# akamiru/bce

Measured on AMD Instinct MI355X. Metric: MB/s compressed, higher is better.
Workload: dtype u8/u32 integer

## Files before the change

bce_amd/csrc/k1_bwt.hip:

```cpp
#include <stdlib.h>

#include <utility>

#include "common.h"
#include "scan_util.h"

namespace bce {

#ifndef K1_ACT_TENTHS
#define K1_ACT_TENTHS 6
#endif

constexpr int K1_T = 256;

constexpr uint32_t K1_MAXB = 1024;
struct K1Plan { uint32_t nb, per_block; };
static K1Plan k1_plan(uint32_t n) {
  const uint32_t chunk = 2048;
  uint32_t chunks = (uint32_t)(((uint64_t)n + chunk - 1) / chunk);
  if (!chunks) chunks = 1;
  uint32_t nb = chunks < K1_MAXB ? chunks : K1_MAXB;
  uint32_t cpb = (chunks + nb - 1) / nb;
  nb = (chunks + cpb - 1) / cpb;
  return {nb, cpb * chunk};
// ... 21 lines not shown
#pragma unroll
    for (uint32_t b = 0; b < 3; ++b) {
      uint64_t q = i + b;
      if (q >= m) q -= m;
      k = (k << 9) | (q == m - 1u ? 0u : (uint32_t)T[q] + 1u);
    }
    keys[i] = k;
    vals[i] = (uint32_t)i;
  }
}

__global__ __launch_bounds__(K1_T) void k1_gather_prev_kernel(const uint32_t *__restrict__ sa,
                                                              const uint32_t *__restrict__ rank, uint32_t n,
                                                              uint32_t h, uint32_t *__restrict__ keys,
                                                              uint32_t *__restrict__ vals) {
  for (uint64_t j = (uint64_t)blockIdx.x * K1_T + threadIdx.x; j < n; j += (uint64_t)gridDim.x * K1_T) {
    const uint32_t q = sa[j];
    const uint32_t p = q >= h ? q - h : q + (n - h);
    vals[j] = p;
    keys[j] = rank[p];
  }
}

__global__ __launch_bounds__(K1_T) void k1_gather_next_kernel(const uint32_t *__restrict__ sa,
                                                              const uint32_t *__restrict__ rank, uint32_t n,
                                                              uint32_t h, uint32_t *__restrict__ k2) {
  for (uint64_t j = (uint64_t)blockIdx.x * K1_T + threadIdx.x; j < n; j += (uint64_t)gridDim.x * K1_T) {
    const uint64_t q = (uint64_t)sa[j] + h;
    k2[j] = rank[q >= n ? q - n : q];
  }
}

__global__ __launch_bounds__(K1_T) void k1_heads_kernel(const uint32_t *__restrict__ k1,
                                                        const uint32_t *__restrict__ k2, uint32_t n,
                                                        uint32_t per_block, uint32_t *__restrict__ nrk,
                                                        uint32_t *__restrict__ blockmax, uint32_t *__restrict__ groups) {
  const uint64_t beg = (uint64_t)blockIdx.x * per_block;
  uint64_t end = beg + per_block;
  if (end > n) end = n;
  uint32_t mx = 0, cnt = 0;
  for (uint64_t j = beg + threadIdx.x; j < end; j += K1_T) {
    bool head = (j == 0);
    if (!head) {
      head = k1[j] != k1[j - 1];
      if (!head && k2) head = k2[j] != k2[j - 1];
    }
    nrk[j] = head ? (uint32_t)j : 0u;
    if (head) { mx = (uint32_t)j; ++cnt; }
  }
  mx = block_reduce_max<K1_T>(mx);
  cnt = block_reduce_sum<K1_T>(cnt);
  if (threadIdx.x == 0) {
    blockmax[blockIdx.x] = mx;
    if (cnt) atomicAdd(groups, cnt);
  }
}

__global__ __launch_bounds__(K1_T) void k1_apply_kernel(const uint32_t *__restrict__ nrk,
                                                        const uint32_t *__restrict__ blockmax, uint32_t n,
                                                        uint32_t per_block, const uint32_t *__restrict__ sa,
                                                        uint32_t *__restrict__ rank) {
  uint32_t c = 0;
  for (uint32_t b = threadIdx.x; b < blockIdx.x; b += K1_T) { const uint32_t v = blockmax[b]; c = c > v ? c : v; }
  uint32_t carry = block_reduce_max<K1_T>(c);
  const uint64_t beg = (uint64_t)blockIdx.x * per_block;
  uint64_t end = beg + per_block;
  if (end > n) end = n;
  for (uint64_t base = beg; base < end; base += K1_T) {
    const uint64_t j = base + threadIdx.x;
    const bool valid = j < end;
    const uint32_t v = valid ? nrk[j] : 0u;
    uint32_t tot;
    uint32_t inc = block_incl_scan_max<K1_T>(v, &tot);
    inc = inc > carry ? inc : carry;
    if (valid) rank[sa[j]] = inc;
    carry = carry > tot ? carry : tot;
  }
}

#ifndef K1_PART_MIN
#define K1_PART_MIN (1u << 27)
#endif

__global__ __launch_bounds__(K1_T) void k1_headidx_kernel(const uint32_t *__restrict__ nrk, const uint32_t *__restrict__ blockmax, uint32_t n,
                                                          uint32_t per_block, uint32_t *__restrict__ hv) {
  uint32_t c = 0;
  for (uint32_t b = threadIdx.x; b < blockIdx.x; b += K1_T) { const uint32_t v = blockmax[b]; c = c > v ? c : v; }
  uint32_t carry = block_reduce_max<K1_T>(c);
  const uint64_t beg = (uint64_t)blockIdx.x * per_block;
  uint64_t end = beg + per_block;
  if (end > n) end = n;
  for (uint64_t base = beg; base < end; base += K1_T) {
    const uint64_t j = base + threadIdx.x;
    const bool valid = j < end;
    const uint32_t v = valid ? nrk[j] : 0u;
    uint32_t tot;
    uint32_t inc = block_incl_scan_max<K1_T>(v, &tot);
    inc = inc > carry ? inc : carry;
    if (valid) hv[j] = inc;
    carry = carry > tot ? carry : tot;
  }
}
__global__ __launch_bounds__(K1_T) void k1_scatter32_kernel(const uint32_t *__restrict__ key, const uint32_t *__restrict__ val, uint32_t m,
                                                            uint32_t limit, uint32_t *__restrict__ dst) {
  for (uint64_t i = (uint64_t)blockIdx.x * K1_T + threadIdx.x; i < m; i += (uint64_t)gridDim.x * K1_T) {
    const uint32_t k = key[i];
    if (k < limit) dst[k] = val[i];
  }
}
__global__ __launch_bounds__(K1_T) void k1_seg_pairs_kernel(const uint32_t *__restrict__ vs, const uint8_t *__restrict__ flag, uint8_t defer, uint32_t m,
                                                            uint32_t *__restrict__ key) {
  for (uint64_t i = (uint64_t)blockIdx.x * K1_T + threadIdx.x; i < m; i += (uint64_t)gridDim.x * K1_T)
    key[i] = (flag[i] & defer) ? 0xFFFFFFFFu : vs[i];
}
__global__ __launch_bounds__(K1_T) void k1_bwt_kernel(const uint8_t *__restrict__ T, const uint32_t *__restrict__ sa,
                                                      uint32_t n, uint8_t *__restrict__ bwt) {
  for (uint64_t j = (uint64_t)blockIdx.x * K1_T + threadIdx.x; j < n; j += (uint64_t)gridDim.x * K1_T) {
    const uint32_t q = sa[j];
    bwt[j] = T[q ? q - 1 : n - 1];
  }
}

__global__ __launch_bounds__(K1_T) void k1_offset_kernel(const uint32_t *__restrict__ rank, uint32_t n,
                                                         uint32_t *__restrict__ out) {
  uint32_t best = 0xFFFFFFFFu;
  for (uint64_t p = (uint64_t)blockIdx.x * K1_T + threadIdx.x; p < n; p += (uint64_t)gridDim.x * K1_T)
    if (rank[p] == 0 && (uint32_t)p < best) best = (uint32_t)p;
#pragma unroll
  for (int o = 32; o > 0; o >>= 1) { const uint32_t t = __shfl_xor(best, o); best = best < t ? best : t; }
  if ((threadIdx.x & 63u) == 0 && best != 0xFFFFFFFFu) atomicMin(out, best);
}


template <int PASS>
__global__ __launch_bounds__(K1_T) void k1_active_kernel(const uint32_t *__restrict__ nrk,
                                                         const uint32_t *__restrict__ src, uint32_t m,
                                                         uint32_t per_block, uint32_t nb, uint32_t *__restrict__ blockcnt,
                                                         uint32_t *__restrict__ out, uint32_t *__restrict__ total, uint32_t mark = 0,
                                                         const uint32_t *__restrict__ sa_in = nullptr, uint32_t *__restrict__ vout = nullptr) {
  const uint64_t beg = (uint64_t)blockIdx.x * per_block;
  uint64_t end = beg + per_block;
  if (end > m) end = m;
  auto keep = [&](uint64_t i) -> bool {
    const bool h0 = i == 0 || nrk[i] != 0;
    const bool h1 = i + 1 >= m || nrk[i + 1] != 0;
    return !(h0 && h1);
  };
  if (PASS == 0) {
    uint32_t c = 0;
    for (uint64_t i = beg + threadIdx.x; i < end; i += K1_T) c += keep(i) ? 1u : 0u;
    c = block_reduce_sum<K1_T>(c);
    if (threadIdx.x == 0) blockcnt[blockIdx.x] = c;
  } else {
    uint32_t b = 0, a = 0;
    for (uint32_t k = threadIdx.x; k < nb; k += K1_T) { const uint32_t v = blockcnt[k]; a += v; if (k < blockIdx.x) b += v; }
    uint32_t base = block_reduce_sum<K1_T>(b);
    const uint32_t all = block_reduce_sum<K1_T>(a);
    if (blockIdx.x == 0 && threadIdx.x == 0) *total = all;
    for (uint64_t c0 = beg; c0 < end; c0 += K1_T) {
      const uint64_t i = c0 + threadIdx.x;
      const bool k = i < end && keep(i);
      uint32_t tot;
      const uint32_t ex = block_excl_scan_sum<K1_T>(k ? 1u : 0u, &tot);
      if (k) {
        out[base + ex] = (src ? src[i] : (uint32_t)i) | ((mark && (i == 0 || nrk[i] != 0)) ? 0x80000000u : 0u);
        if (vout) vout[base + ex] = sa_in[i];
      }
      base += tot;
    }
  }
}

__global__ __launch_bounds__(K1_T) void k1_act_gather_kernel(const uint32_t *__restrict__ A, const uint32_t *__restrict__ sa,
                                                             const uint32_t *__restrict__ rank, uint32_t n, uint32_t m,
                                                             uint32_t h, uint32_t *__restrict__ keys,
                                                             uint32_t *__restrict__ vals) {
  for (uint64_t i = (uint64_t)blockIdx.x * K1_T + threadIdx.x; i < m; i += (uint64_t)gridDim.x * K1_T) {
    const uint32_t p = sa[A[i]];
    const uint64_t q = (uint64_t)p + h;
    vals[i] = p;
    keys[i] = rank[q >= n ? q - n : q];
  }
}
__global__ __launch_bounds__(K1_T) void k1_act_group_kernel(const uint32_t *__restrict__ vals,
                                                            const uint32_t *__restrict__ rank, uint32_t m,
// ... 278 lines not shown
      }
      if (big) {
        if (w < SEG_CH) { flag[i] = KF_DEFER; ++ndef; }
      } else if (g0 >= SEG_CAP && g0 < SEG_CAP + SEG_CH) {
        mine[it] = true; gs[it] = g0 - SEG_CAP; ge[it] = g1 - SEG_CAP;
      }
    }
  }
#pragma unroll
  for (int it = 0; it < EPT; ++it) if (mine[it]) sfx[it] = V[base + it * SEG_T + (int)tid];
#pragma unroll
  for (int it = 0; it < EPT; ++it)
    if (mine[it]) {
      uint64_t q = (uint64_t)sfx[it] + h;
      if (q >= n) q -= n;
      k2[it] = rank[q];
    }
#pragma unroll
  for (int it = 0; it < EPT; ++it) if (mine[it]) K[it * SEG_T + (int)tid] = k2[it];
  if (ndef) atomicAdd(&s_defer, ndef);
  __syncthreads();
  int pos[EPT];
#pragma unroll
  for (int it = 0; it < EPT; ++it) {
    pos[it] = 0;
    if (mine[it]) {
      const int w = it * SEG_T + (int)tid;
      const uint32_t kw = k2[it];
      uint32_t r = 0;
      {
        int t = gs[it];
        const int e = w;
        for (; t < e && (t & 3); ++t) r += K[t] <= kw ? 1u : 0u;
        for (; t + 4 <= e; t += 4) {
          const uint4 v = *reinterpret_cast<const uint4 *>(&K[t]);
          r += (v.x <= kw ? 1u : 0u) + (v.y <= kw ? 1u : 0u) + (v.z <= kw ? 1u : 0u) + (v.w <= kw ? 1u : 0u);
        }
        for (; t < e; ++t) r += K[t] <= kw ? 1u : 0u;
      }
      {
        int t = w + 1;
        const int e = ge[it];
        for (; t < e && (t & 3); ++t) r += K[t] < kw ? 1u : 0u;
        for (; t + 4 <= e; t += 4) {
          const uint4 v = *reinterpret_cast<const uint4 *>(&K[t]);
          r += (v.x < kw ? 1u : 0u) + (v.y < kw ? 1u : 0u) + (v.z < kw ? 1u : 0u) + (v.w < kw ? 1u : 0u);
        }
        for (; t < e; ++t) r += K[t] < kw ? 1u : 0u;
      }
      pos[it] = gs[it] + (int)r;
    }
  }
  __syncthreads();
#pragma unroll
  for (int it = 0; it < EPT; ++it) if (mine[it]) { K[pos[it]] = k2[it]; S[pos[it]] = sfx[it]; }
  __syncthreads();
#pragma unroll
  for (int it = 0; it < EPT; ++it) {
    const int w = it * SEG_T + (int)tid;
    if ((w & ~63) < cntw) {
      const bool nh = mine[it] && (w == gs[it] || K[w] != K[w - 1]);
      const uint64_t bal = __ballot(nh);
      if (lane == 0) nbits[w >> 6] = bal;
    }
  }
  __syncthreads();
#pragma unroll
  for (int it = 0; it < EPT; ++it)
    if (mine[it]) {
      const int w = it * SEG_T + (int)tid;
      const int hp = seg_prev_bit(nbits, w, gs[it]);
      const bool nh = hp == w;
      const bool next_head = (w + 1 == ge[it]) || ((nbits[(w + 1) >> 6] >> ((w + 1) & 63)) & 1ull);
      const int64_t i = base + w;
      const uint32_t s = S[w];
      sa[SL[w]] = s;
      nr[i] = SL[hp];
      vs[i] = s;
      flag[i] = (uint8_t)((nh ? KF_HEAD : 0) | ((nh && next_head) ? 0 : KF_KEEP));
    }
  if (tid == 0 && s_defer) atomicAdd(ndefer, s_defer);
}

__global__ __launch_bounds__(K1_T) void k1_seg_apply_kernel(const uint32_t *__restrict__ nr, const uint32_t *__restrict__ vs,
                                                            const uint8_t *__restrict__ flag, uint32_t m, uint32_t *__restrict__ rank) {
  for (uint64_t i = (uint64_t)blockIdx.x * K1_T + threadIdx.x; i < m; i += (uint64_t)gridDim.x * K1_T)
    if (!(flag[i] & KF_DEFER)) rank[vs[i]] = nr[i];
}

template <int PASS, int MODE>
__global__ __launch_bounds__(K1_T) void k1_relist_kernel(const uint32_t *__restrict__ A, const uint32_t *__restrict__ vs,
                                                         const uint8_t *__restrict__ flag, uint32_t m,
                                                         uint32_t per_block, uint32_t nb, uint32_t *__restrict__ blockcnt,
                                                         uint32_t *__restrict__ out, uint32_t *__restrict__ out2, uint32_t *__restrict__ total,
                                                         uint32_t *__restrict__ blockcnt2 = nullptr, uint32_t *__restrict__ out3 = nullptr) {
  const uint64_t beg = (uint64_t)blockIdx.x * per_block;
  uint64_t end = beg + per_block;
  if (end > m) end = m;
  auto take = [&](uint64_t i) -> bool { return MODE == 0 ? (flag[i] & KF_DEFER) != 0 : (flag[i] & KF_KEEP) != 0; };
  if (PASS == 0) {
    uint32_t cnt = 0, hc = 0;
    for (uint64_t i = beg + threadIdx.x; i < end; i += K1_T) {
      const bool k = take(i);
      cnt += k ? 1u : 0u;
      if (MODE == 0) hc += (k && (A[i] & K1_HEAD)) ? 1u : 0u;
    }
    cnt = block_reduce_sum<K1_T>(cnt);
    if (MODE == 0) hc = block_reduce_sum<K1_T>(hc);
    if (threadIdx.x == 0) { blockcnt[blockIdx.x] = cnt; if (MODE == 0) blockcnt2[blockIdx.x] = hc; }
  } else {
    uint32_t b = 0, a = 0, b2 = 0, a2 = 0;
    for (uint32_t k = threadIdx.x; k < nb; k += K1_T) {
      const uint32_t v = blockcnt[k];
      a += v; if (k < blockIdx.x) b += v;
      if (MODE == 0) { const uint32_t v2 = blockcnt2[k]; a2 += v2; if (k < blockIdx.x) b2 += v2; }
    }
    uint32_t base = block_reduce_sum<K1_T>(b);
    const uint32_t all = block_reduce_sum<K1_T>(a);
    uint32_t hbase = 0;
    if (MODE == 0) {
      hbase = block_reduce_sum<K1_T>(b2);
      const uint32_t all2 = block_reduce_sum<K1_T>(a2);
      if (blockIdx.x == 0 && threadIdx.x == 0) total[1] = all2;
    }
    if (blockIdx.x == 0 && threadIdx.x == 0) total[0] = all;
    for (uint64_t c0 = beg; c0 < end; c0 += K1_T) {
      const uint64_t i = c0 + threadIdx.x;
      const bool k = i < end && take(i);
      const uint32_t a_i = (MODE == 0 && k) ? A[i] : 0u;
      uint32_t tot;
      const uint32_t ex = block_excl_scan_sum<K1_T>(k ? 1u : 0u, &tot);
      uint32_t htot = 0, hex = 0;
      const uint32_t hd = (MODE == 0 && (a_i & K1_HEAD)) ? 1u : 0u;
      if (MODE == 0) hex = block_excl_scan_sum<K1_T>(hd, &htot);
      if (k) {
        if (MODE == 0) { out[base + ex] = (uint32_t)i; out2[base + ex] = a_i & K1_SLOT; out3[base + ex] = hbase + hex + hd - 1u; }
        else { out[base + ex] = (A[i] & K1_SLOT) | ((flag[i] & KF_HEAD) ? K1_HEAD : 0u); out2[base + ex] = vs[i]; }
      }
      base += tot;
      hbase += htot;
    }
  }
}

__global__ __launch_bounds__(K1_T) void k1_big_gather_kernel(const uint32_t *__restrict__ idx, const uint32_t *__restrict__ gid,
                                                             const uint32_t *__restrict__ V, const uint32_t *__restrict__ rank,
                                                             uint32_t n, uint32_t nd, uint32_t h, uint32_t rbits,
                                                             uint32_t *__restrict__ lo, uint32_t *__restrict__ hi, uint32_t *__restrict__ val) {
  for (uint64_t j = (uint64_t)blockIdx.x * K1_T + threadIdx.x; j < nd; j += (uint64_t)gridDim.x * K1_T) {
    const uint32_t p = V[idx[j]];
    uint64_t q = (uint64_t)p + h;
    if (q >= n) q -= n;
    const uint64_t key = ((uint64_t)gid[j] << rbits) | rank[q];
    lo[j] = (uint32_t)key;
    hi[j] = (uint32_t)(key >> 32);
    val[j] = p;
  }
}
__global__ __launch_bounds__(K1_T) void k1_big_heads_kernel(const uint32_t *__restrict__ slots, const uint32_t *__restrict__ lo,
                                                            const uint32_t *__restrict__ hi, const uint32_t *__restrict__ val,
                                                            uint32_t nd, uint32_t per_block, uint32_t *__restrict__ sa,
                                                            uint32_t *__restrict__ nrk, uint32_t *__restrict__ blockmax) {
  const uint64_t beg = (uint64_t)blockIdx.x * per_block;
  uint64_t end = beg + per_block;
  if (end > nd) end = nd;
  uint32_t mx = 0;
  for (uint64_t j = beg + threadIdx.x; j < end; j += K1_T) {
    const uint32_t slot = slots[j];
    sa[slot] = val[j];
    const bool head = j == 0 || lo[j] != lo[j - 1] || hi[j] != hi[j - 1];
    nrk[j] = head ? slot : 0u;
    if (head) mx = slot;
  }
  mx = block_reduce_max<K1_T>(mx);
  if (threadIdx.x == 0) blockmax[blockIdx.x] = mx;
}

__global__ __launch_bounds__(K1_T) void k1_defer_flags_kernel(const uint32_t *__restrict__ nrk, const uint32_t *__restrict__ idx,
                                                              const uint32_t *__restrict__ sorted, uint32_t nd,
                                                              uint8_t *__restrict__ flag, uint32_t *__restrict__ vs) {
  for (uint64_t j = (uint64_t)blockIdx.x * K1_T + threadIdx.x; j < nd; j += (uint64_t)gridDim.x * K1_T) {
    const bool hd = j == 0 || nrk[j] != 0u;
    const bool nx = j + 1 >= nd || nrk[j + 1] != 0u;
    const uint32_t i = idx[j];
    flag[i] = (uint8_t)(KF_DEFER | (hd ? KF_HEAD : 0) | ((hd && nx) ? 0 : KF_KEEP));
    vs[i] = sorted[j];
  }
}

static int k1_sort_rotations(bce_hip_ctx *c, const uint8_t *T, uint32_t n, bool sentinel) {
  if (getenv("BCE_K1_V1")) return k1_sort_rotations_v1(c, T, n, sentinel);
  const size_t b4 = (size_t)n * 4;
  for (int i = 0; i < 2; ++i) { BCE_TRY(ensure(c, c->sa[i], b4)); BCE_TRY(ensure(c, c->key[i], b4)); BCE_TRY(ensure(c, c->khi[i], b4)); }
  BCE_TRY(ensure(c, c->rank, b4));
  BCE_TRY(ensure(c, c->k2, b4));
  BCE_TRY(ensure(c, c->nrk, b4));
  BCE_TRY(ensure(c, c->kflag, (size_t)n + 16));
  for (int i = 0; i < 2; ++i) { BCE_TRY(ensure(c, c->act[i], b4)); BCE_TRY(ensure(c, c->actv[i], b4)); }
  const K1Plan pl = k1_plan(n);
  BCE_TRY(ensure(c, c->blk, (size_t)(K1_MAXB + K1_SC_CODE + 128 + K1_MAXB) * 4));
  uint32_t *blockmax = c->blk.as<uint32_t>();
  uint32_t *scalars = blockmax + K1_MAXB;
  uint32_t *rank = c->rank.as<uint32_t>(), *k2 = c->k2.as<uint32_t>(), *nrk = c->nrk.as<uint32_t>();
  uint8_t *flag = c->kflag.as<uint8_t>();
  const uint32_t g = grid_for(n);
  const bool trace = getenv("BCE_K1_TRACE") != nullptr;
  double t_prev = now_s();
  auto lap = [&](const char *what, uint64_t h, uint32_t m, uint32_t nd) {
    if (!trace) return;
    (void)hipStreamSynchronize(c->stream);
    const double t = now_s();
    fprintf(stderr, "k1 %p: %-10s h %llu active %u deferred %u (+%.2f ms)\n", (void *)c, what, (unsigned long long)h, m, nd, (t - t_prev) * 1e3);
    t_prev = t;
  };

  const uint32_t nbytes = sentinel ? n - 1u : n;
  BCE_HIP_TRY(c, hipMemsetAsync(scalars + K1_SC_HIST, 0, 256 * 4, c->stream));
  hipLaunchKernelGGL(k1_bytehist_kernel, dim3(g < 1024u ? g : 1024u), dim3(K1_T), 0, c->stream, T, nbytes, scalars + K1_SC_HIST);
  uint32_t hist[256];
  BCE_TRY(read_back(c, hist, scalars + K1_SC_HIST, sizeof hist));
  uint16_t code[256];
  uint32_t sigma = sentinel ? 1u : 0u;
  for (int b = 0; b < 256; ++b) { code[b] = (uint16_t)sigma; if (hist[b]) ++sigma; }
  uint32_t bits = ceil_log2(sigma);
  if (bits < 1) bits = 1;
  uint32_t nsym = 64u / bits;
  if (nsym > 16u) nsym = 16u;
  if (const char *e = getenv("BCE_K1_KEYBITS")) { const uint32_t v = (uint32_t)strtoul(e, nullptr, 10); if (v >= bits && v / bits < nsym) nsym = v / bits; }
  const uint32_t keybits = nsym * bits;
  {
    if (!c->h_small) BCE_TRY(pin_alloc(c, &c->h_small, 4096));
    memcpy(c->h_small, code, sizeof code);
    BCE_HIP_TRY(c, hipMemcpyAsync(scalars + K1_SC_CODE, c->h_small, sizeof code, hipMemcpyHostToDevice, c->stream));
  }

  uint32_t *lo[2] = {c->key[0].as<uint32_t>(), c->key[1].as<uint32_t>()};
  uint32_t *hi[2] = {c->khi[0].as<uint32_t>(), c->khi[1].as<uint32_t>()};
  uint32_t *val[2] = {c->sa[0].as<uint32_t>(), c->sa[1].as<uint32_t>()};
  {
    const uint32_t per = K1_T * K1I_E;
    hipLaunchKernelGGL(k1_init64_kernel, dim3((uint32_t)(((uint64_t)n + per - 1) / per)), dim3(K1_T), 0, c->stream, T, n, nbytes,
                       reinterpret_cast<const uint16_t *>(scalars + K1_SC_CODE), bits, nsym, lo[0], hi[0], val[0]);
  }
  int res = 0;
  BCE_TRY(radix_sort_wide(c, lo, hi, val, n, keybits, &res, 9));
  lap("first sort", nsym, n, 0);
  BCE_HIP_TRY(c, hipMemsetAsync(scalars, 0, 16, c->stream));
  hipLaunchKernelGGL(k1_heads_kernel, dim3(pl.nb), dim3(K1_T), 0, c->stream, hi[res], lo[res], n, pl.per_block, nrk, blockmax, scalars);
  const uint32_t rbits = ceil_log2(n);
  static const uint32_t part_min = getenv("BCE_K1_PART_MIN") ? (uint32_t)strtoul(getenv("BCE_K1_PART_MIN"), nullptr, 10) : K1_PART_MIN;
  const bool sorted_apply = n >= part_min;
  if (sorted_apply) hipLaunchKernelGGL(k1_headidx_kernel, dim3(pl.nb), dim3(K1_T), 0, c->stream, nrk, blockmax, n, pl.per_block, k2);
  else hipLaunchKernelGGL(k1_apply_kernel, dim3(pl.nb), dim3(K1_T), 0, c->stream, nrk, blockmax, n, pl.per_block, val[res], rank);
  uint32_t *act[2] = {c->act[0].as<uint32_t>(), c->act[1].as<uint32_t>()};
  uint32_t *actv[2] = {c->actv[0].as<uint32_t>(), c->actv[1].as<uint32_t>()};
  uint32_t m = 0;
  hipLaunchKernelGGL(k1_active_kernel<0>, dim3(pl.nb), dim3(K1_T), 0, c->stream, nrk, (const uint32_t *)nullptr, n, pl.per_block, pl.nb,
                     blockmax, act[0], scalars + 2, 1u, (const uint32_t *)val[res], actv[0]);
  hipLaunchKernelGGL(k1_active_kernel<1>, dim3(pl.nb), dim3(K1_T), 0, c->stream, nrk, (const uint32_t *)nullptr, n, pl.per_block, pl.nb,
                     blockmax, act[0], scalars + 2, 1u, (const uint32_t *)val[res], actv[0]);
  if (sorted_apply) {
    const uint32_t b1 = rbits / ((rbits + 9u) / 10u);
    uint32_t *pk[2] = {val[res], lo[res ^ 1]}, *pv[2] = {k2, rank};
    int pr = 0;
    BCE_TRY(radix_sort_pairs(c, pk, pv, n, 0, b1, &pr, 10));
    uint32_t *qk[2] = {lo[res ^ 1], hi[res ^ 1]}, *qv[2] = {rank, val[res ^ 1]};
    BCE_TRY(radix_sort_pairs(c, qk, qv, n, b1, rbits - b1, &pr, 10));
    if (pr) BCE_HIP_TRY(c, hipMemcpyAsync(rank, qv[1], (size_t)n * 4, hipMemcpyDeviceToDevice, c->stream));
  }
  BCE_TRY(read_back(c, &m, scalars + 2, 4));
  lap("first ranks", nsym, m, 0);

  uint64_t h = nsym;
  uint32_t *sa = val[res];
  uint32_t *nr = hi[0], *vs = hi[1];
  while (m > 0 && h < n) {
    const uint32_t *A = act[0];
    const uint32_t nblk = (uint32_t)(((uint64_t)m + SEG_CH - 1) / SEG_CH);
    BCE_HIP_TRY(c, hipMemsetAsync(scalars + 3, 0, 4, c->stream));
    hipLaunchKernelGGL(k1_seg_sort_kernel, dim3(nblk), dim3(SEG_T), 0, c->stream, A, (const uint32_t *)actv[0], m, sa, rank, n, (uint32_t)h, nr, vs,
                       flag, scalars + 3);
    uint32_t nd = 0;
    BCE_TRY(read_back(c, &nd, scalars + 3, 4));
    const K1Plan ap = k1_plan(m);
    if (nd) {
      BCE_TRY(ensure(c, c->dl[0], (size_t)nd * 4));
      BCE_TRY(ensure(c, c->dl[1], (size_t)nd * 4));
      BCE_TRY(ensure(c, c->dl[2], (size_t)nd * 4));
      BCE_TRY(ensure(c, c->dl[3], (size_t)nd * 4));
      uint32_t *idx = c->dl[0].as<uint32_t>(), *slots = c->dl[1].as<uint32_t>(), *gid = c->dl[2].as<uint32_t>();
      uint32_t *blockcnt2 = scalars + K1_SC_CODE + 128;
      hipLaunchKernelGGL((k1_relist_kernel<0, 0>), dim3(ap.nb), dim3(K1_T), 0, c->stream, A, (const uint32_t *)vs, flag, m, ap.per_block, ap.nb, blockmax, idx, slots,
                         scalars + 4, blockcnt2, gid);
      hipLaunchKernelGGL((k1_relist_kernel<1, 0>), dim3(ap.nb), dim3(K1_T), 0, c->stream, A, (const uint32_t *)vs, flag, m, ap.per_block, ap.nb, blockmax, idx, slots,
                         scalars + 4, blockcnt2, gid);
      uint32_t cnts[2] = {0, 0};
      BCE_TRY(read_back(c, cnts, scalars + 4, 8));
      if (cnts[0] != nd || cnts[1] == 0 || cnts[1] > nd) { snprintf(c->err, sizeof c->err, "k1: deferred list %u / %u groups, expected %u elements", cnts[0], cnts[1], nd); return BCE_HIP_E_INTERNAL; }
      const uint32_t gbits = ceil_log2(cnts[1]);
      uint32_t *bl[2] = {lo[0], lo[1]};
      uint32_t *bh[2] = {val[res ^ 1], k2};
      uint32_t *bv[2] = {nrk, c->dl[3].as<uint32_t>()};
      const uint32_t ga = grid_for(nd);
      hipLaunchKernelGGL(k1_big_gather_kernel, dim3(ga), dim3(K1_T), 0, c->stream, idx, gid, (const uint32_t *)actv[0], rank, n, nd, (uint32_t)h, rbits,
                         bl[0], bh[0], bv[0]);
      int rb = 0;
      BCE_TRY(radix_sort_wide(c, bl, bh, bv, nd, rbits + gbits, &rb, 9));
      const K1Plan dp = k1_plan(nd);
      uint32_t *snrk = bv[rb ^ 1];
      hipLaunchKernelGGL(k1_big_heads_kernel, dim3(dp.nb), dim3(K1_T), 0, c->stream, slots, bl[rb], bh[rb], bv[rb], nd, dp.per_block, sa, snrk, blockmax);
      hipLaunchKernelGGL(k1_act_apply_kernel, dim3(dp.nb), dim3(K1_T), 0, c->stream, snrk, blockmax, nd, dp.per_block, bv[rb], rank);
      uint32_t *vjr = bv[rb];
      hipLaunchKernelGGL(k1_defer_flags_kernel, dim3(ga), dim3(K1_T), 0, c->stream, snrk, idx, (const uint32_t *)vjr, nd, flag, vs);
    }
    if (m >= part_min) {
      const uint32_t b1 = rbits / ((rbits + 9u) / 10u);
      uint32_t *pk[2] = {lo[0], lo[1]}, *pv[2] = {nr, k2};
      hipLaunchKernelGGL(k1_seg_pairs_kernel, dim3(grid_for(m)), dim3(K1_T), 0, c->stream, (const uint32_t *)vs, (const uint8_t *)flag, KF_DEFER, m, pk[0]);
      int pr = 0;
      BCE_TRY(radix_sort_pairs(c, pk, pv, m, 0, b1, &pr, 10));
      uint32_t *qk[2] = {lo[1], lo[0]}, *qv[2] = {k2, val[res ^ 1]};
      BCE_TRY(radix_sort_pairs(c, qk, qv, m, b1, rbits - b1, &pr, 10));
      hipLaunchKernelGGL(k1_scatter32_kernel, dim3(grid_for(m)), dim3(K1_T), 0, c->stream, (const uint32_t *)qk[pr], (const uint32_t *)qv[pr], m, n, rank);
    } else {
      hipLaunchKernelGGL(k1_seg_apply_kernel, dim3(grid_for(m)), dim3(K1_T), 0, c->stream, nr, vs, flag, m, rank);
    }
    hipLaunchKernelGGL((k1_relist_kernel<0, 1>), dim3(ap.nb), dim3(K1_T), 0, c->stream, A, (const uint32_t *)vs, flag, m, ap.per_block, ap.nb, blockmax, act[1],
                       actv[1], scalars + 2);
    hipLaunchKernelGGL((k1_relist_kernel<1, 1>), dim3(ap.nb), dim3(K1_T), 0, c->stream, A, (const uint32_t *)vs, flag, m, ap.per_block, ap.nb, blockmax, act[1],
                       actv[1], scalars + 2);
    const uint32_t m_old = m;
    BCE_TRY(read_back(c, &m, scalars + 2, 4));
    std::swap(act[0], act[1]);
    std::swap(actv[0], actv[1]);
    h <<= 1;
    c->stats.sort_rounds++;
    lap("round", h, m, nd);
    (void)m_old;
  }
  BCE_HIP_TRY(c, hipGetLastError());
  c->k1_unique = m == 0;
  c->sa_res = res;
  return BCE_HIP_OK;
}

int k1_bwt(bce_hip_ctx *c) {
  const uint32_t n = c->n;
  uint8_t *T = c->text.as<uint8_t>();
  BCE_TRY(ensure(c, c->bwt, n));
  uint8_t *bwt = c->bwt.as<uint8_t>();
  c->stats.sort_rounds = 0;
  c->k1_unique = false;
  c->k1_valid = false;
  if (n == 1) {
    BCE_HIP_TRY(c, hipMemcpyAsync(bwt, T, 1, hipMemcpyDeviceToDevice, c->stream));
    BCE_HIP_TRY(c, hipStreamSynchronize(c->stream));
    c->offset = 0;
    return BCE_HIP_OK;
  }
  BCE_TRY(k1_sort_rotations(c, T, n, false));
  const uint32_t g = grid_for(n);
  uint32_t *scalars = c->blk.as<uint32_t>() + K1_MAXB;
  const uint32_t *sa = c->sa[c->sa_res].as<uint32_t>();
  BCE_HIP_TRY(c, hipMemsetAsync(scalars + 1, 0xFF, 4, c->stream));
  hipLaunchKernelGGL(k1_bwt_kernel, dim3(g), dim3(K1_T), 0, c->stream, T, sa, n, bwt);
  hipLaunchKernelGGL(k1_offset_kernel, dim3(g), dim3(K1_T), 0, c->stream, c->rank.as<uint32_t>(), n, scalars + 1);
  uint32_t off = 0;
  BCE_TRY(read_back(c, &off, scalars + 1, 4));
  BCE_HIP_TRY(c, hipGetLastError());
  if (off >= n) { snprintf(c->err, sizeof c->err, "k1: no rank-0 rotation found"); return BCE_HIP_E_INTERNAL; }
  c->offset = off;
  c->k1_valid = true;
  return BCE_HIP_OK;
}

__global__ __launch_bounds__(K1_T) void k1_divbwt_gather_kernel(const uint8_t *__restrict__ T, const uint32_t *__restrict__ sa,
                                                                uint32_t m, uint32_t pidx, uint8_t *__restrict__ U) {
  for (uint64_t j = (uint64_t)blockIdx.x * K1_T + threadIdx.x; j < m; j += (uint64_t)gridDim.x * K1_T) {
    const uint32_t p = sa[j];
    if (p != 0u) U[j < pidx ? j : j - 1u] = T[p - 1u];
  }
}

int k1_divbwt(bce_hip_ctx *c, const uint8_t *T_host, uint8_t *U_host, uint32_t n, uint32_t *pidx_out) {
  if (n == 0 || n >= 0x7FFFFFFFu) return BCE_HIP_E_ARG;
  const uint32_t m = n + 1u;
  c->stage = 0; c->k1_valid = false; c->enum_active = false; c->text_loaded = false;
  BCE_TRY(ensure(c, c->text, m));
  BCE_TRY(ensure(c, c->bwt, m));
  uint8_t *T = c->text.as<uint8_t>();
  BCE_HIP_TRY(c, hipMemcpyAsync(T, T_host, n, hipMemcpyHostToDevice, c->stream));
  c->stats.sort_rounds = 0;
  BCE_TRY(k1_sort_rotations(c, T, m, true));
  uint32_t pidx = 0;
  BCE_TRY(read_back(c, &pidx, c->rank.as<uint32_t>(), 4));
  if (pidx == 0 || pidx > n) { snprintf(c->err, sizeof c->err, "divbwt: primary index %u out of range", pidx); return BCE_HIP_E_INTERNAL; }
  hipLaunchKernelGGL(k1_divbwt_gather_kernel, dim3(grid_for(m)), dim3(K1_T), 0, c->stream, T, c->sa[c->sa_res].as<uint32_t>(), m,
                     pidx, c->bwt.as<uint8_t>());
  BCE_HIP_TRY(c, hipMemcpyAsync(U_host, c->bwt.p, n, hipMemcpyDeviceToHost, c->stream));
  BCE_HIP_TRY(c, hipStreamSynchronize(c->stream));
  BCE_HIP_TRY(c, hipGetLastError());
  *pidx_out = pidx;
  return BCE_HIP_OK;
}

}
```

Baseline: 839.8.

## Fuse first-rank kernels and round relist/apply, cutting host read-backs per round

Builds the symbol code table on the GPU, so the host no longer reads back the histogram and uploads the table. It replaces the heads, headidx/apply and active kernels of the first round with a count pass plus one fused apply pass that computes head keys in place. In each doubling round it fuses the rank apply into the relist, uses a popcount-based count kernel, and speculatively relists guarded on the deferred count. When nothing is deferred, one synchronisation point per round is dropped. The cost is more complex kernels and guard-based early exits that must behave correctly when the speculation is discarded.

```diff
diff --git a/bce_amd/csrc/k1_bwt.hip b/bce_amd/csrc/k1_bwt.hip
--- a/bce_amd/csrc/k1_bwt.hip
+++ b/bce_amd/csrc/k1_bwt.hip
@@ -127,25 +127,6 @@
 #define K1_PART_MIN (1u << 27)
 #endif
 
-__global__ __launch_bounds__(K1_T) void k1_headidx_kernel(const uint32_t *__restrict__ nrk, const uint32_t *__restrict__ blockmax, uint32_t n,
-                                                          uint32_t per_block, uint32_t *__restrict__ hv) {
-  uint32_t c = 0;
-  for (uint32_t b = threadIdx.x; b < blockIdx.x; b += K1_T) { const uint32_t v = blockmax[b]; c = c > v ? c : v; }
-  uint32_t carry = block_reduce_max<K1_T>(c);
-  const uint64_t beg = (uint64_t)blockIdx.x * per_block;
-  uint64_t end = beg + per_block;
-  if (end > n) end = n;
-  for (uint64_t base = beg; base < end; base += K1_T) {
-    const uint64_t j = base + threadIdx.x;
-    const bool valid = j < end;
-    const uint32_t v = valid ? nrk[j] : 0u;
-    uint32_t tot;
-    uint32_t inc = block_incl_scan_max<K1_T>(v, &tot);
-    inc = inc > carry ? inc : carry;
-    if (valid) hv[j] = inc;
-    carry = carry > tot ? carry : tot;
-  }
-}
 __global__ __launch_bounds__(K1_T) void k1_scatter32_kernel(const uint32_t *__restrict__ key, const uint32_t *__restrict__ val, uint32_t m,
                                                             uint32_t limit, uint32_t *__restrict__ dst) {
   for (uint64_t i = (uint64_t)blockIdx.x * K1_T + threadIdx.x; i < m; i += (uint64_t)gridDim.x * K1_T) {
@@ -590,61 +571,45 @@
   if (tid == 0 && s_defer) atomicAdd(ndefer, s_defer);
 }
 
-__global__ __launch_bounds__(K1_T) void k1_seg_apply_kernel(const uint32_t *__restrict__ nr, const uint32_t *__restrict__ vs,
-                                                            const uint8_t *__restrict__ flag, uint32_t m, uint32_t *__restrict__ rank) {
-  for (uint64_t i = (uint64_t)blockIdx.x * K1_T + threadIdx.x; i < m; i += (uint64_t)gridDim.x * K1_T)
-    if (!(flag[i] & KF_DEFER)) rank[vs[i]] = nr[i];
-}
-
-template <int PASS, int MODE>
-__global__ __launch_bounds__(K1_T) void k1_relist_kernel(const uint32_t *__restrict__ A, const uint32_t *__restrict__ vs,
-                                                         const uint8_t *__restrict__ flag, uint32_t m,
-                                                         uint32_t per_block, uint32_t nb, uint32_t *__restrict__ blockcnt,
-                                                         uint32_t *__restrict__ out, uint32_t *__restrict__ out2, uint32_t *__restrict__ total,
-                                                         uint32_t *__restrict__ blockcnt2 = nullptr, uint32_t *__restrict__ out3 = nullptr) {
+template <int PASS>
+__global__ __launch_bounds__(K1_T) void k1_defer_list_kernel(const uint32_t *__restrict__ A, const uint8_t *__restrict__ flag, uint32_t m,
+                                                             uint32_t per_block, uint32_t nb, uint32_t *__restrict__ blockcnt,
+                                                             uint32_t *__restrict__ blockcnt2, uint32_t *__restrict__ idx,
+                                                             uint32_t *__restrict__ slots, uint32_t *__restrict__ gid, uint32_t *__restrict__ total) {
   const uint64_t beg = (uint64_t)blockIdx.x * per_block;
   uint64_t end = beg + per_block;
   if (end > m) end = m;
-  auto take = [&](uint64_t i) -> bool { return MODE == 0 ? (flag[i] & KF_DEFER) != 0 : (flag[i] & KF_KEEP) != 0; };
   if (PASS == 0) {
     uint32_t cnt = 0, hc = 0;
     for (uint64_t i = beg + threadIdx.x; i < end; i += K1_T) {
-      const bool k = take(i);
+      const bool k = (flag[i] & KF_DEFER) != 0;
       cnt += k ? 1u : 0u;
-      if (MODE == 0) hc += (k && (A[i] & K1_HEAD)) ? 1u : 0u;
+      hc += (k && (A[i] & K1_HEAD)) ? 1u : 0u;
     }
     cnt = block_reduce_sum<K1_T>(cnt);
-    if (MODE == 0) hc = block_reduce_sum<K1_T>(hc);
-    if (threadIdx.x == 0) { blockcnt[blockIdx.x] = cnt; if (MODE == 0) blockcnt2[blockIdx.x] = hc; }
+    hc = block_reduce_sum<K1_T>(hc);
+    if (threadIdx.x == 0) { blockcnt[blockIdx.x] = cnt; blockcnt2[blockIdx.x] = hc; }
   } else {
     uint32_t b = 0, a = 0, b2 = 0, a2 = 0;
     for (uint32_t k = threadIdx.x; k < nb; k += K1_T) {
-      const uint32_t v = blockcnt[k];
-      a += v; if (k < blockIdx.x) b += v;
-      if (MODE == 0) { const uint32_t v2 = blockcnt2[k]; a2 += v2; if (k < blockIdx.x) b2 += v2; }
+      const uint32_t v = blockcnt[k], v2 = blockcnt2[k];
+      a += v; a2 += v2;
+      if (k < blockIdx.x) { b += v; b2 += v2; }
     }
     uint32_t base = block_reduce_sum<K1_T>(b);
     const uint32_t all = block_reduce_sum<K1_T>(a);
-    uint32_t hbase = 0;
-    if (MODE == 0) {
-      hbase = block_reduce_sum<K1_T>(b2);
-      const uint32_t all2 = block_reduce_sum<K1_T>(a2);
-      if (blockIdx.x == 0 && threadIdx.x == 0) total[1] = all2;
-    }
-    if (blockIdx.x == 0 && threadIdx.x == 0) total[0] = all;
+    uint32_t hbase = block_reduce_sum<K1_T>(b2);
+    const uint32_t all2 = block_reduce_sum<K1_T>(a2);
+    if (blockIdx.x == 0 && threadIdx.x == 0) { total[0] = all; total[1] = all2; }
     for (uint64_t c0 = beg; c0 < end; c0 += K1_T) {
       const uint64_t i = c0 + threadIdx.x;
-      const bool k = i < end && take(i);
-      const uint32_t a_i = (MODE == 0 && k) ? A[i] : 0u;
-      uint32_t tot;
+      const bool k = i < end && (flag[i] & KF_DEFER) != 0;
+      const uint32_t a_i = k ? A[i] : 0u;
+      const uint32_t hd = (a_i & K1_HEAD) ? 1u : 0u;
+      uint32_t tot, htot;
       const uint32_t ex = block_excl_scan_sum<K1_T>(k ? 1u : 0u, &tot);
-      uint32_t htot = 0, hex = 0;
-      const uint32_t hd = (MODE == 0 && (a_i & K1_HEAD)) ? 1u : 0u;
-      if (MODE == 0) hex = block_excl_scan_sum<K1_T>(hd, &htot);
-      if (k) {
-        if (MODE == 0) { out[base + ex] = (uint32_t)i; out2[base + ex] = a_i & K1_SLOT; out3[base + ex] = hbase + hex + hd - 1u; }
-        else { out[base + ex] = (A[i] & K1_SLOT) | ((flag[i] & KF_HEAD) ? K1_HEAD : 0u); out2[base + ex] = vs[i]; }
-      }
+      const uint32_t hex = block_excl_scan_sum<K1_T>(hd, &htot);
+      if (k) { idx[base + ex] = (uint32_t)i; slots[base + ex] = a_i & K1_SLOT; gid[base + ex] = hbase + hex + hd - 1u; }
       base += tot;
       hbase += htot;
     }
@@ -696,6 +661,126 @@
   }
 }
 
+__global__ __launch_bounds__(K1_T) void k1_codetable_kernel(const uint32_t *__restrict__ hist, uint32_t first, uint16_t *__restrict__ code,
+                                                            uint32_t *__restrict__ sigma) {
+  uint32_t tot;
+  const uint32_t ex = block_excl_scan_sum<K1_T>(hist[threadIdx.x] ? 1u : 0u, &tot);
+  code[threadIdx.x] = (uint16_t)(first + ex);
+  if (threadIdx.x == 0) *sigma = first + tot;
+}
+
+__device__ __forceinline__ void k1_key_heads(const uint32_t *__restrict__ hi, const uint32_t *__restrict__ lo, uint64_t j, uint64_t end,
+                                             uint32_t n, bool valid, bool *head, bool *nhead) {
+  const uint32_t lane = threadIdx.x & 63u;
+  auto key = [&](uint64_t q) -> uint64_t { return ((uint64_t)hi[q] << 32) | lo[q]; };
+  const uint64_t k = valid ? key(j) : 0ull;
+  uint64_t kp = __shfl_up(k, 1), kn = __shfl_down(k, 1);
+  if (valid && lane == 0 && j > 0) kp = key(j - 1);
+  if (valid && (lane == 63 || j + 1 >= end) && j + 1 < n) kn = key(j + 1);
+  *head = valid && (j == 0 || k != kp);
+  *nhead = valid && (j + 1 >= n || k != kn);
+}
+
+__global__ __launch_bounds__(K1_T) void k1_first_count_kernel(const uint32_t *__restrict__ hi, const uint32_t *__restrict__ lo, uint32_t n,
+                                                              uint32_t per_block, uint32_t *__restrict__ blockmax,
+                                                              uint32_t *__restrict__ blockcnt) {
+  const uint64_t beg = (uint64_t)blockIdx.x * per_block;
+  uint64_t end = beg + per_block;
+  if (end > n) end = n;
+  uint32_t mx = 0, cnt = 0;
+  for (uint64_t base = beg; base < end; base += K1_T) {
+    const uint64_t j = base + threadIdx.x;
+    bool head, nhead;
+    k1_key_heads(hi, lo, j, end, n, j < end, &head, &nhead);
+    if (head) mx = (uint32_t)j;
+    cnt += (j < end && !(head && nhead)) ? 1u : 0u;
+  }
+  mx = block_reduce_max<K1_T>(mx);
+  cnt = block_reduce_sum<K1_T>(cnt);
+  if (threadIdx.x == 0) { blockmax[blockIdx.x] = mx; blockcnt[blockIdx.x] = cnt; }
+}
+
+template <bool SCATTER>
+__global__ __launch_bounds__(K1_T) void k1_first_apply_kernel(const uint32_t *__restrict__ hi, const uint32_t *__restrict__ lo,
+                                                              const uint32_t *__restrict__ sa, uint32_t n, uint32_t per_block, uint32_t nb,
+                                                              const uint32_t *__restrict__ blockmax, const uint32_t *__restrict__ blockcnt,
+                                                              uint32_t *__restrict__ dst, uint32_t *__restrict__ act,
+                                                              uint32_t *__restrict__ actv, uint32_t *__restrict__ total) {
+  uint32_t c = 0, b = 0, a = 0;
+  for (uint32_t k = threadIdx.x; k < nb; k += K1_T) {
+    const uint32_t v = blockcnt[k];
+    a += v;
+    if (k < blockIdx.x) { b += v; const uint32_t x = blockmax[k]; c = c > x ? c : x; }
+  }
+  uint32_t carry = block_reduce_max<K1_T>(c);
+  uint32_t lbase = block_reduce_sum<K1_T>(b);
+  const uint32_t all = block_reduce_sum<K1_T>(a);
+  if (blockIdx.x == 0 && threadIdx.x == 0) *total = all;
+  const uint64_t beg = (uint64_t)blockIdx.x * per_block;
+  uint64_t end = beg + per_block;
+  if (end > n) end = n;
+  for (uint64_t base = beg; base < end; base += K1_T) {
+    const uint64_t j = base + threadIdx.x;
+    const bool valid = j < end;
+    bool head, nhead;
+    k1_key_heads(hi, lo, j, end, n, valid, &head, &nhead);
+    const bool keep = valid && !(head && nhead);
+    const uint32_t s = valid ? sa[j] : 0u;
+    uint32_t tot, ktot;
+    uint32_t inc = block_incl_scan_max<K1_T>(head ? (uint32_t)j : 0u, &tot);
+    inc = inc > carry ? inc : carry;
+    const uint32_t ex = block_excl_scan_sum<K1_T>(keep ? 1u : 0u, &ktot);
+    if (valid) dst[SCATTER ? s : (uint32_t)j] = inc;
+    if (keep) { act[lbase + ex] = (uint32_t)j | (head ? K1_HEAD : 0u); actv[lbase + ex] = s; }
+    carry = carry > tot ? carry : tot;
+    lbase += ktot;
+  }
+}
+
+__global__ __launch_bounds__(K1_T) void k1_round_count_kernel(const uint8_t *__restrict__ flag, uint32_t m, uint32_t per_block,
+                                                              uint32_t *__restrict__ blockcnt, const uint32_t *__restrict__ guard) {
+  if (guard && *guard) return;
+  const uint64_t beg = (uint64_t)blockIdx.x * per_block;
+  uint64_t end = beg + per_block;
+  if (end > m) end = m;
+  uint32_t cnt = 0;
+  for (uint64_t i = beg + 4ull * threadIdx.x; i < end; i += 4ull * K1_T) {
+    uint32_t w = *reinterpret_cast<const uint32_t *>(flag + i) & (0x01010101u * KF_KEEP);
+    if (end - i < 4) w &= 0xFFFFFFFFu >> (8u * (4u - (uint32_t)(end - i)));
+    cnt += (uint32_t)__popc(w);
+  }
+  cnt = block_reduce_sum<K1_T>(cnt);
+  if (threadIdx.x == 0) blockcnt[blockIdx.x] = cnt;
+}
+template <bool APPLY>
+__global__ __launch_bounds__(K1_T) void k1_round_apply_kernel(const uint32_t *__restrict__ A, const uint32_t *__restrict__ nr,
+                                                              const uint32_t *__restrict__ vs, const uint8_t *__restrict__ flag, uint32_t m,
+                                                              uint32_t per_block, uint32_t nb, const uint32_t *__restrict__ blockcnt,
+                                                              uint32_t *__restrict__ rank, uint32_t *__restrict__ out, uint32_t *__restrict__ out2,
+                                                              uint32_t *__restrict__ total, const uint32_t *__restrict__ guard) {
+  if (guard && *guard) return;
+  uint32_t b = 0, a = 0;
+  for (uint32_t k = threadIdx.x; k < nb; k += K1_T) { const uint32_t v = blockcnt[k]; a += v; if (k < blockIdx.x) b += v; }
+  uint32_t base = block_reduce_sum<K1_T>(b);
+  const uint32_t all = block_reduce_sum<K1_T>(a);
+  if (blockIdx.x == 0 && threadIdx.x == 0) *total = all;
+  const uint64_t beg = (uint64_t)blockIdx.x * per_block;
+  uint64_t end = beg + per_block;
+  if (end > m) end = m;
+  for (uint64_t c0 = beg; c0 < end; c0 += K1_T) {
+    const uint64_t i = c0 + threadIdx.x;
+    const uint8_t f = i < end ? flag[i] : (uint8_t)0;
+    const bool k = (f & KF_KEEP) != 0;
+    const bool ap = APPLY && i < end && !(f & KF_DEFER);
+    const uint32_t s = (k || ap) ? vs[i] : 0u;
+    if (ap) rank[s] = nr[i];
+    uint32_t tot;
+    const uint32_t ex = block_excl_scan_sum<K1_T>(k ? 1u : 0u, &tot);
+    if (k) { out[base + ex] = (A[i] & K1_SLOT) | ((f & KF_HEAD) ? K1_HEAD : 0u); out2[base + ex] = s; }
+    base += tot;
+  }
+}
+
 static int k1_sort_rotations(bce_hip_ctx *c, const uint8_t *T, uint32_t n, bool sentinel) {
   if (getenv("BCE_K1_V1")) return k1_sort_rotations_v1(c, T, n, sentinel);
   const size_t b4 = (size_t)n * 4;
@@ -709,6 +794,7 @@
   BCE_TRY(ensure(c, c->blk, (size_t)(K1_MAXB + K1_SC_CODE + 128 + K1_MAXB) * 4));
   uint32_t *blockmax = c->blk.as<uint32_t>();
   uint32_t *scalars = blockmax + K1_MAXB;
+  uint32_t *blockcnt2 = scalars + K1_SC_CODE + 128;
   uint32_t *rank = c->rank.as<uint32_t>(), *k2 = c->k2.as<uint32_t>(), *nrk = c->nrk.as<uint32_t>();
   uint8_t *flag = c->kflag.as<uint8_t>();
   const uint32_t g = grid_for(n);
@@ -721,26 +807,22 @@
     fprintf(stderr, "k1 %p: %-10s h %llu active %u deferred %u (+%.2f ms)\n", (void *)c, what, (unsigned long long)h, m, nd, (t - t_prev) * 1e3);
     t_prev = t;
   };
+  uint32_t waits = 0;
+  auto fetch = [&](void *dst, const uint32_t *src, size_t bytes) -> int { ++waits; return read_back(c, dst, src, bytes); };
 
   const uint32_t nbytes = sentinel ? n - 1u : n;
   BCE_HIP_TRY(c, hipMemsetAsync(scalars + K1_SC_HIST, 0, 256 * 4, c->stream));
   hipLaunchKernelGGL(k1_bytehist_kernel, dim3(g < 1024u ? g : 1024u), dim3(K1_T), 0, c->stream, T, nbytes, scalars + K1_SC_HIST);
-  uint32_t hist[256];
-  BCE_TRY(read_back(c, hist, scalars + K1_SC_HIST, sizeof hist));
-  uint16_t code[256];
-  uint32_t sigma = sentinel ? 1u : 0u;
-  for (int b = 0; b < 256; ++b) { code[b] = (uint16_t)sigma; if (hist[b]) ++sigma; }
+  hipLaunchKernelGGL(k1_codetable_kernel, dim3(1), dim3(K1_T), 0, c->stream, (const uint32_t *)(scalars + K1_SC_HIST), sentinel ? 1u : 0u,
+                     reinterpret_cast<uint16_t *>(scalars + K1_SC_CODE), scalars + 6);
+  uint32_t sigma = 0;
+  BCE_TRY(fetch(&sigma, scalars + 6, 4));
   uint32_t bits = ceil_log2(sigma);
   if (bits < 1) bits = 1;
   uint32_t nsym = 64u / bits;
   if (nsym > 16u) nsym = 16u;
   if (const char *e = getenv("BCE_K1_KEYBITS")) { const uint32_t v = (uint32_t)strtoul(e, nullptr, 10); if (v >= bits && v / bits < nsym) nsym = v / bits; }
   const uint32_t keybits = nsym * bits;
-  {
-    if (!c->h_small) BCE_TRY(pin_alloc(c, &c->h_small, 4096));
-    memcpy(c->h_small, code, sizeof code);
-    BCE_HIP_TRY(c, hipMemcpyAsync(scalars + K1_SC_CODE, c->h_small, sizeof code, hipMemcpyHostToDevice, c->stream));
-  }
 
   uint32_t *lo[2] = {c->key[0].as<uint32_t>(), c->key[1].as<uint32_t>()};
   uint32_t *hi[2] = {c->khi[0].as<uint32_t>(), c->khi[1].as<uint32_t>()};
@@ -753,21 +835,18 @@
   int res = 0;
   BCE_TRY(radix_sort_wide(c, lo, hi, val, n, keybits, &res, 9));
   lap("first sort", nsym, n, 0);
-  BCE_HIP_TRY(c, hipMemsetAsync(scalars, 0, 16, c->stream));
-  hipLaunchKernelGGL(k1_heads_kernel, dim3(pl.nb), dim3(K1_T), 0, c->stream, hi[res], lo[res], n, pl.per_block, nrk, blockmax, scalars);
   const uint32_t rbits = ceil_log2(n);
   static const uint32_t part_min = getenv("BCE_K1_PART_MIN") ? (uint32_t)strtoul(getenv("BCE_K1_PART_MIN"), nullptr, 10) : K1_PART_MIN;
   const bool sorted_apply = n >= part_min;
-  if (sorted_apply) hipLaunchKernelGGL(k1_headidx_kernel, dim3(pl.nb), dim3(K1_T), 0, c->stream, nrk, blockmax, n, pl.per_block, k2);
-  else hipLaunchKernelGGL(k1_apply_kernel, dim3(pl.nb), dim3(K1_T), 0, c->stream, nrk, blockmax, n, pl.per_block, val[res], rank);
   uint32_t *act[2] = {c->act[0].as<uint32_t>(), c->act[1].as<uint32_t>()};
   uint32_t *actv[2] = {c->actv[0].as<uint32_t>(), c->actv[1].as<uint32_t>()};
   uint32_t m = 0;
-  hipLaunchKernelGGL(k1_active_kernel<0>, dim3(pl.nb), dim3(K1_T), 0, c->stream, nrk, (const uint32_t *)nullptr, n, pl.per_block, pl.nb,
-                     blockmax, act[0], scalars + 2, 1u, (const uint32_t *)val[res], actv[0]);
-  hipLaunchKernelGGL(k1_active_kernel<1>, dim3(pl.nb), dim3(K1_T), 0, c->stream, nrk, (const uint32_t *)nullptr, n, pl.per_block, pl.nb,
-                     blockmax, act[0], scalars + 2, 1u, (const uint32_t *)val[res], actv[0]);
+  hipLaunchKernelGGL(k1_first_count_kernel, dim3(pl.nb), dim3(K1_T), 0, c->stream, (const uint32_t *)hi[res], (const uint32_t *)lo[res], n, pl.per_block,
+                     blockmax, blockcnt2);
   if (sorted_apply) {
+    hipLaunchKernelGGL(k1_first_apply_kernel<false>, dim3(pl.nb), dim3(K1_T), 0, c->stream, (const uint32_t *)hi[res], (const uint32_t *)lo[res],
+                       (const uint32_t *)val[res], n, pl.per_block, pl.nb, (const uint32_t *)blockmax, (const uint32_t *)blockcnt2, k2, act[0], actv[0],
+                       scalars + 2);
     const uint32_t b1 = rbits / ((rbits + 9u) / 10u);
     uint32_t *pk[2] = {val[res], lo[res ^ 1]}, *pv[2] = {k2, rank};
     int pr = 0;
@@ -775,8 +854,12 @@
     uint32_t *qk[2] = {lo[res ^ 1], hi[res ^ 1]}, *qv[2] = {rank, val[res ^ 1]};
     BCE_TRY(radix_sort_pairs(c, qk, qv, n, b1, rbits - b1, &pr, 10));
     if (pr) BCE_HIP_TRY(c, hipMemcpyAsync(rank, qv[1], (size_t)n * 4, hipMemcpyDeviceToDevice, c->stream));
-  }
-  BCE_TRY(read_back(c, &m, scalars + 2, 4));
+  } else {
+    hipLaunchKernelGGL(k1_first_apply_kernel<true>, dim3(pl.nb), dim3(K1_T), 0, c->stream, (const uint32_t *)hi[res], (const uint32_t *)lo[res],
+                       (const uint32_t *)val[res], n, pl.per_block, pl.nb, (const uint32_t *)blockmax, (const uint32_t *)blockcnt2, rank, act[0], actv[0],
+                       scalars + 2);
+  }
+  BCE_TRY(fetch(&m, scalars + 2, 4));
   lap("first ranks", nsym, m, 0);
 
   uint64_t h = nsym;
@@ -788,22 +871,40 @@
     BCE_HIP_TRY(c, hipMemsetAsync(scalars + 3, 0, 4, c->stream));
     hipLaunchKernelGGL(k1_seg_sort_kernel, dim3(nblk), dim3(SEG_T), 0, c->stream, A, (const uint32_t *)actv[0], m, sa, rank, n, (uint32_t)h, nr, vs,
                        flag, scalars + 3);
-    uint32_t nd = 0;
-    BCE_TRY(read_back(c, &nd, scalars + 3, 4));
     const K1Plan ap = k1_plan(m);
+    const bool sorted_round = m >= part_min;
+    auto relist = [&](const uint32_t *guard) {
+      hipLaunchKernelGGL(k1_round_count_kernel, dim3(ap.nb), dim3(K1_T), 0, c->stream, (const uint8_t *)flag, m, ap.per_block, blockmax, guard);
+      if (sorted_round)
+        hipLaunchKernelGGL(k1_round_apply_kernel<false>, dim3(ap.nb), dim3(K1_T), 0, c->stream, A, (const uint32_t *)nr, (const uint32_t *)vs,
+                           (const uint8_t *)flag, m, ap.per_block, ap.nb, (const uint32_t *)blockmax, rank, act[1], actv[1], scalars + 2, guard);
+      else
+        hipLaunchKernelGGL(k1_round_apply_kernel<true>, dim3(ap.nb), dim3(K1_T), 0, c->stream, A, (const uint32_t *)nr, (const uint32_t *)vs,
+                           (const uint8_t *)flag, m, ap.per_block, ap.nb, (const uint32_t *)blockmax, rank, act[1], actv[1], scalars + 2, guard);
+    };
+    uint32_t nd = 0, m_next = 0;
+    bool listed = false;
+    if (!sorted_round) {
+      relist(scalars + 3);
+      uint32_t two[2] = {0, 0};
+      BCE_TRY(fetch(two, scalars + 2, 8));
+      m_next = two[0]; nd = two[1];
+      listed = nd == 0;
+    } else {
+      BCE_TRY(fetch(&nd, scalars + 3, 4));
+    }
     if (nd) {
       BCE_TRY(ensure(c, c->dl[0], (size_t)nd * 4));
       BCE_TRY(ensure(c, c->dl[1], (size_t)nd * 4));
       BCE_TRY(ensure(c, c->dl[2], (size_t)nd * 4));
       BCE_TRY(ensure(c, c->dl[3], (size_t)nd * 4));
       uint32_t *idx = c->dl[0].as<uint32_t>(), *slots = c->dl[1].as<uint32_t>(), *gid = c->dl[2].as<uint32_t>();
-      uint32_t *blockcnt2 = scalars + K1_SC_CODE + 128;
-      hipLaunchKernelGGL((k1_relist_kernel<0, 0>), dim3(ap.nb), dim3(K1_T), 0, c->stream, A, (const uint32_t *)vs, flag, m, ap.per_block, ap.nb, blockmax, idx, slots,
-                         scalars + 4, blockcnt2, gid);
-      hipLaunchKernelGGL((k1_relist_kernel<1, 0>), dim3(ap.nb), dim3(K1_T), 0, c->stream, A, (const uint32_t *)vs, flag, m, ap.per_block, ap.nb, blockmax, idx, slots,
-                         scalars + 4, blockcnt2, gid);
+      hipLaunchKernelGGL(k1_defer_list_kernel<0>, dim3(ap.nb), dim3(K1_T), 0, c->stream, A, (const uint8_t *)flag, m, ap.per_block, ap.nb, blockmax, blockcnt2,
+                         idx, slots, gid, scalars + 4);
+      hipLaunchKernelGGL(k1_defer_list_kernel<1>, dim3(ap.nb), dim3(K1_T), 0, c->stream, A, (const uint8_t *)flag, m, ap.per_block, ap.nb, blockmax, blockcnt2,
+                         idx, slots, gid, scalars + 4);
       uint32_t cnts[2] = {0, 0};
-      BCE_TRY(read_back(c, cnts, scalars + 4, 8));
+      BCE_TRY(fetch(cnts, scalars + 4, 8));
       if (cnts[0] != nd || cnts[1] == 0 || cnts[1] > nd) { snprintf(c->err, sizeof c->err, "k1: deferred list %u / %u groups, expected %u elements", cnts[0], cnts[1], nd); return BCE_HIP_E_INTERNAL; }
       const uint32_t gbits = ceil_log2(cnts[1]);
       uint32_t *bl[2] = {lo[0], lo[1]};
@@ -821,32 +922,29 @@
       uint32_t *vjr = bv[rb];
       hipLaunchKernelGGL(k1_defer_flags_kernel, dim3(ga), dim3(K1_T), 0, c->stream, snrk, idx, (const uint32_t *)vjr, nd, flag, vs);
     }
-    if (m >= part_min) {
-      const uint32_t b1 = rbits / ((rbits + 9u) / 10u);
-      uint32_t *pk[2] = {lo[0], lo[1]}, *pv[2] = {nr, k2};
-      hipLaunchKernelGGL(k1_seg_pairs_kernel, dim3(grid_for(m)), dim3(K1_T), 0, c->stream, (const uint32_t *)vs, (const uint8_t *)flag, KF_DEFER, m, pk[0]);
-      int pr = 0;
-      BCE_TRY(radix_sort_pairs(c, pk, pv, m, 0, b1, &pr, 10));
-      uint32_t *qk[2] = {lo[1], lo[0]}, *qv[2] = {k2, val[res ^ 1]};
-      BCE_TRY(radix_sort_pairs(c, qk, qv, m, b1, rbits - b1, &pr, 10));
-      hipLaunchKernelGGL(k1_scatter32_kernel, dim3(grid_for(m)), dim3(K1_T), 0, c->stream, (const uint32_t *)qk[pr], (const uint32_t *)qv[pr], m, n, rank);
-    } else {
-      hipLaunchKernelGGL(k1_seg_apply_kernel, dim3(grid_for(m)), dim3(K1_T), 0, c->stream, nr, vs, flag, m, rank);
-    }
-    hipLaunchKernelGGL((k1_relist_kernel<0, 1>), dim3(ap.nb), dim3(K1_T), 0, c->stream, A, (const uint32_t *)vs, flag, m, ap.per_block, ap.nb, blockmax, act[1],
-                       actv[1], scalars + 2);
-    hipLaunchKernelGGL((k1_relist_kernel<1, 1>), dim3(ap.nb), dim3(K1_T), 0, c->stream, A, (const uint32_t *)vs, flag, m, ap.per_block, ap.nb, blockmax, act[1],
-                       actv[1], scalars + 2);
-    const uint32_t m_old = m;
-    BCE_TRY(read_back(c, &m, scalars + 2, 4));
+    if (!listed) {
+      if (sorted_round) {
+        const uint32_t b1 = rbits / ((rbits + 9u) / 10u);
+        uint32_t *pk[2] = {lo[0], lo[1]}, *pv[2] = {nr, k2};
+        hipLaunchKernelGGL(k1_seg_pairs_kernel, dim3(grid_for(m)), dim3(K1_T), 0, c->stream, (const uint32_t *)vs, (const uint8_t *)flag, KF_DEFER, m, pk[0]);
+        int pr = 0;
+        BCE_TRY(radix_sort_pairs(c, pk, pv, m, 0, b1, &pr, 10));
+        uint32_t *qk[2] = {lo[1], lo[0]}, *qv[2] = {k2, val[res ^ 1]};
+        BCE_TRY(radix_sort_pairs(c, qk, qv, m, b1, rbits - b1, &pr, 10));
+        hipLaunchKernelGGL(k1_scatter32_kernel, dim3(grid_for(m)), dim3(K1_T), 0, c->stream, (const uint32_t *)qk[pr], (const uint32_t *)qv[pr], m, n, rank);
+      }
+      relist(nullptr);
+      BCE_TRY(fetch(&m_next, scalars + 2, 4));
+    }
+    m = m_next;
     std::swap(act[0], act[1]);
     std::swap(actv[0], actv[1]);
     h <<= 1;
     c->stats.sort_rounds++;
     lap("round", h, m, nd);
-    (void)m_old;
   }
   BCE_HIP_TRY(c, hipGetLastError());
+  if (trace) fprintf(stderr, "k1 %p: %u read-backs in the sort\n", (void *)c, waits);
   c->k1_unique = m == 0;
   c->sa_res = res;
   return BCE_HIP_OK;
```

Result: slower. 829.6 (-1.2%).
